# lamm-mit/MoleculeDiffusionTransformer

Hardware: AMD Instinct MI355X
Metric: molecules/sec @64 diffusion steps (QM9 max_len=64) (higher is better)
Workload: dtype f32 storage/accumulate; GEMM products as split-bf16 (bf16x3) MFMA; 1 GPU; QMDiffusion inverse sample(): channels=64 pred_dim=16 max_len=64 cond_len=12, batch=1024/GPU, 64 timesteps (126 U-Net evals), cond_scale=1.0, fp32; global_batch=1024, parallelism=batch-shard x1

## Files before the change

moleculediffusiontransformer_amd/csrc/k_tf256.hip:

```cpp
#include <cstdlib>
#include <type_traits>

#include "mdt_kernels.h"
#include "mdt_device.h"

#ifndef MDT_TF_F32
#define MDT_TF_F32 0
#endif

#ifndef MDT_KV_CPOL
#define MDT_KV_CPOL 2
#endif

namespace mdt {

namespace {

enum { K_T = 0, K_N = 1, K_O = 2 };
enum { D_P = 0, D_O = 1, D_K = 2, D_V = 3, D_SCRATCH = 4, D_SCRATCH_VEC = 5 };

template <int N>
__device__ __forceinline__ void frag_wait() {
#ifdef MDT_ABL_LGKM
  __builtin_amdgcn_sched_barrier(0);
#else
  lgkm_wait<N>();
#endif
}

constexpr int C = 256;
constexpr int CS = 128;
constexpr int SLOT = 256 * CS;
constexpr int NS = 4;
constexpr int IPT = CS / 16;
constexpr int NST = C / 32;
constexpr int NCT = C / 16;
constexpr int NU = 4;
constexpr int KTM = 3;
constexpr int RED_BYTES = KTM * 4 * 64 * 16;
constexpr int VEC_FLOATS = 768;
constexpr int VEC_BYTES = VEC_FLOATS * 4;
#ifndef MDT_XH_MODE
#define MDT_XH_MODE 0
#endif
#ifdef MDT_ABL_BAR
#define MDT_BARRIER() __builtin_amdgcn_sched_barrier(0)
#else
#define MDT_BARRIER() __builtin_amdgcn_s_barrier()
#endif
#ifndef MDT_STREAM_PF
#define MDT_STREAM_PF 8
#endif
#ifndef MDT_RING_AHEAD
#define MDT_RING_AHEAD 2
#endif
#ifndef MDT_XH_ADDR
#define MDT_XH_ADDR 1
#endif
constexpr int AUX_ST = MDT_XH_MODE == 1 ? 17 : (MDT_XH_MODE == 3 ? 18 : (MDT_XH_MODE == 4 ? 19 : 16));
constexpr int AUX_LD = MDT_XH_MODE == 0 ? 16 : (MDT_XH_MODE == 3 ? 18 : (MDT_XH_MODE == 4 ? 19 : 17));
constexpr unsigned XBLOCK = 32 * C * 4;
constexpr unsigned long long POLL_TIMEOUT = 30000000ull;

}

template <int NPW, int NSPLIT, bool F32>
__global__ __launch_bounds__(512) void k_tf256(TFArgs a) {
  extern __shared__ __attribute__((aligned(1024))) unsigned char smem[];
  unsigned char* red_b = smem + NS * SLOT;
  unsigned char* vec_b = red_b + RED_BYTES;

  const int tid = threadIdx.x, lane = tid & 63;
  const int wave = __builtin_amdgcn_readfirstlane(tid >> 6);
  const int NT = a.NT;
  const unsigned char* wsrc = reinterpret_cast<const unsigned char*>(a.w);
  int rb = blockIdx.x, hh = 0;
  const int nrb = (a.M + 31) / 32;
  if constexpr (NSPLIT == 2) {
    const int S = a.pair_stride, id = blockIdx.x;
    const int grp = id / (2 * S), w = id - grp * 2 * S;
    hh = w / S;
    rb = a.rb_base + grp * S + (w - hh * S);
    if (rb >= nrb) return;
  }

  if (wave >= 4) {
    const int iw = wave - 4;
    __builtin_amdgcn_s_setprio(MDT_LOADER_PRIO);
    const cu32p tiles = (cu32p)(a.tiles + (NSPLIT == 2 ? hh * NT : 0));
    const int lpP = lane >> 5;
    const int xP = (lane & 15) ^ lpP;
    const int baseP = ((lane >> 4) & 1) * (128 * CS) + lpP * (2 * CS);
    const int xO = (lane & 7) ^ (lane >> 4);
    const int baseO = (lane >> 3) * 128;
    unsigned voffP[IPT], voffO[IPT];
#pragma unroll
    for (int q = 0; q < IPT; ++q) {
      const int inst = iw + 4 * q;
      const int U = 2 * inst;
      voffP[q] = F32 ? (unsigned)(inst * 1024 + lane * 16) : (unsigned)(U * (2 * CS) + ((xP ^ (U & 15)) << 4) + baseP);
      voffO[q] = F32 ? (unsigned)(inst * 1024 + lane * 16)
                     : (unsigned)(((inst * 8) / CS) * (128 * CS) + ((inst * 8) % CS) * 128 + ((xO ^ (4 * (inst & 1))) << 4) + baseO);
    }
    const int sample0 = rb * (32 / a.T);
    const bool second = a.kv2 && sample0 >= a.nsamples / 2;
    unsigned voffKV[8];
    if constexpr (NPW > 0) {
      const int kv_rows = (32 / a.T) * a.Tk;
      const int bstr = second ? 0 : a.kv_bstride;
#pragma unroll
      for (int q = 0; q < NPW; ++q) {
        const int R = 4 * (iw + 4 * q) + (lane >> 4);
        const int Rc = min(R, kv_rows - 1);
        const int sm = min(Rc / a.Tk, a.nsamples - 1 - sample0), key = Rc % a.Tk;
        voffKV[q] = (unsigned)(((sm * bstr + key) * a.ldkv + 4 * ((lane & 15) ^ (R & 15))) * 4);
      }
    }
    auto pieces_of = [&](unsigned d) -> int {
      const unsigned kind = d & 7u;
      if (kind == D_SCRATCH) return 0;
      if (kind == D_SCRATCH_VEC) return iw < VEC_BYTES / 1024 ? 1 : 0;
      if (kind >= D_K) return NPW;
      return IPT;
    };
    auto issue_vec = [&](unsigned aux) {
      if (iw < VEC_BYTES / 1024)
        __builtin_amdgcn_global_load_lds(reinterpret_cast<const unsigned char*>(a.vec) + (aux >> 1) * 1024 + iw * 1024 + lane * 16,
                                         (__attribute__((address_space(3))) void*)(vec_b + (aux & 1u) * VEC_BYTES + iw * 1024), 16, 0, 0);
    };
    auto issue_tile = [&](int tau, unsigned d) {
      unsigned char* slot = smem + MDT_SLOT_IDX(tau) * SLOT + iw * 1024;
      const unsigned kind = d & 7u, aux = d >> 3;
      if (kind == D_SCRATCH) return;
      if (kind == D_SCRATCH_VEC) { issue_vec(aux); return; }
      if (kind >= D_K) {
        if constexpr (NPW > 0) {
          const int layer = (int)(aux >> 4), head = (int)(aux & 15u);
          const float* lb = second ? a.kv2 + (int64_t)layer * a.kv2_lstride
                                   : a.kv + (int64_t)layer * a.kv_lstride + (int64_t)sample0 * a.kv_bstride * a.ldkv;
          const unsigned char* base = reinterpret_cast<const unsigned char*>(lb + 64 * head + (kind == D_V ? 64 * a.nheads : 0));
#pragma unroll
          for (int q = 0; q < NPW; ++q)
            __builtin_amdgcn_global_load_lds(base + voffKV[q], (__attribute__((address_space(3))) void*)(slot + q * 4096), 16, 0, MDT_KV_CPOL);
        }
        return;
      }
      const unsigned char* tile = wsrc + (int64_t)aux * SLOT;
      const bool ptile = kind == D_P;
#pragma unroll
      for (int q = 0; q < IPT; ++q) {
        const unsigned off = ptile ? voffP[q] : voffO[q];
        __builtin_amdgcn_global_load_lds(tile + off, (__attribute__((address_space(3))) void*)(slot + q * 4096), 16, 0, 0);
      }
    };
    auto wait_vm = [&](int allow) {
#ifdef MDT_ABL_VMWAIT
      return;
#endif
      switch (allow) {
#define MDT_VMW(n) case n: asm volatile("s_waitcnt vmcnt(" #n ")" ::: "memory"); break;
        MDT_VMW(0) MDT_VMW(1) MDT_VMW(2) MDT_VMW(3) MDT_VMW(4) MDT_VMW(5) MDT_VMW(6) MDT_VMW(7) MDT_VMW(8) MDT_VMW(9) MDT_VMW(10)
        MDT_VMW(11) MDT_VMW(12) MDT_VMW(13) MDT_VMW(14) MDT_VMW(15)
#undef MDT_VMW
        default: asm volatile("s_waitcnt vmcnt(16)" ::: "memory"); break;
      }
    };
    constexpr int AHEAD = MDT_RING_AHEAD;
    unsigned dq[AHEAD];
    MDT_BARRIER();
    issue_vec(0u);
#pragma unroll
    for (int j = 0; j < AHEAD; ++j) {
      const unsigned d = j < NT ? tiles[j] : 0u;
      if (j < NT) issue_tile(j, d);
      if (j > 0) dq[j - 1] = d;
    }
    constexpr bool PF_ON = MDT_STREAM_PF > 0 && AHEAD == 2;
    const int pf_groups = PF_ON ? max(1, (int)gridDim.x / (8 * NSPLIT)) : 1;
    const int pf_mine = (int)blockIdx.x / (8 * NSPLIT);
    int pf_turn = MDT_STREAM_PF % pf_groups;
    unsigned char* pf_sink_b = vec_b + 2 * VEC_BYTES;
    int pf1 = 0, pf2 = 0;
    for (int k = 0; k < NT; ++k) {
      const unsigned dnew = k + AHEAD < NT ? tiles[k + AHEAD] : 0u;
      int allow = 0;
#pragma unroll
      for (int j = 0; j < AHEAD - 1; ++j) allow += k + 1 + j < NT ? pieces_of(dq[j]) : 0;
      if (PF_ON && k + 1 < NT) allow += pf1 + pf2;
      if (allow == IPT) asm volatile("s_waitcnt vmcnt(8)" ::: "memory");
      else if (NPW > 0 && allow == NPW) asm volatile("s_waitcnt vmcnt(%0)" ::"n"(NPW > 0 ? NPW : 1) : "memory");
      else wait_vm(allow);
      MDT_BARRIER();
      if (k + AHEAD < NT) issue_tile(k + AHEAD, dnew);
      if constexpr (PF_ON) {
        pf2 = pf1;
        pf1 = 0;
        const bool mine = pf_turn == pf_mine;
        if (++pf_turn == pf_groups) pf_turn = 0;
        if (mine && k + MDT_STREAM_PF < NT) {
          const unsigned dp = tiles[k + MDT_STREAM_PF];
          const unsigned kp = dp & 7u;
          if (kp != D_SCRATCH && kp != D_SCRATCH_VEC && kp < D_K) {
            const unsigned char* t = wsrc + (int64_t)(dp >> 3) * SLOT + (iw * 64 + lane) * 128;
            __builtin_amdgcn_global_load_lds(t, (__attribute__((address_space(3))) void*)(pf_sink_b + iw * 256), 4, 0, 0);
            pf1 = 1;
          }
        }
      }
#pragma unroll
      for (int j = 0; j + 1 < AHEAD - 1; ++j) dq[j] = dq[j + 1];
      dq[AHEAD - 2] = dnew;
    }
    prefetch_next_weights(a.pf_ptr, a.pf_lines, iw * 64 + lane);
    return;
  }

  const int i = lane & 15, g = lane >> 4;
  const int rt = wave >> 1, fh = wave & 1;
  const int row0 = rb * 32 + rt * 16;
  const int m = row0 + i;
  const bool mvalid = m < a.M;
  const int mc = mvalid ? m : a.M - 1;
  f32x4* red = reinterpret_cast<f32x4*>(red_b);

  f32x4 accT[NCT];
#ifdef MDT_STAMPS
  unsigned long long* stamps = reinterpret_cast<unsigned long long*>(a.xflags + 64 + 64 * nrb + 512 * hh);
  int nstamp = 0;
#define MDT_STAMP()                                                                                           \
  do {                                                                                                        \
    if (NSPLIT == 2 && rb == 0 && wave == 0 && nstamp < 250) {                                                \
      unsigned long long t_;                                                                                  \
      asm volatile("s_memtime %0\n\ts_waitcnt lgkmcnt(0)" : "=s"(t_)::"memory");                              \
      if (lane == 0) stamps[nstamp] = (t_ & 0xffffffffffffull) | ((unsigned long long)__LINE__ << 48);        \
      ++nstamp;                                                                                               \
    }                                                                                                         \
  } while (0)
#else
#define MDT_STAMP() do {} while (0)
#endif
#ifdef MDT_XH_LOG
  unsigned xlog_first = 0, xlog_last = 0, xlog_got = 0, xlog_epoch = 0;
#endif
  unsigned xround = 0;
  int xn = 0;
  __amdgpu_buffer_rsrc_t xres, fres;
  const unsigned fown = (64u + 32u * (unsigned)(2 * rb + hh)) * 4u;
  if constexpr (NSPLIT == 2) {
    xres = __builtin_amdgcn_make_buffer_rsrc(a.xbuf, 0, 0x7fffffff, 0x00020000);
    fres = __builtin_amdgcn_make_buffer_rsrc(a.xflags, 0, 0x7fffffff, 0x00020000);
    xround = (unsigned)__builtin_amdgcn_readfirstlane(__builtin_amdgcn_raw_buffer_load_b32(fres, fown, 0, AUX_LD));
  }
#ifdef MDT_XH_LOG
  xlog_epoch = xround;
#endif
  {
    const float* xp = a.x + (int64_t)mc * C + 4 * g;
    float4 xr[NCT];
#pragma unroll
    for (int ct = 0; ct < NCT; ++ct) xr[ct] = *reinterpret_cast<const float4*>(xp + 16 * ct);
    __builtin_amdgcn_sched_barrier(0);
    MDT_BARRIER();
    __builtin_amdgcn_sched_barrier(0);
#pragma unroll
    for (int ct = 0; ct < NCT; ++ct) accT[ct] = f32x4{xr[ct].x, xr[ct].y, xr[ct].z, xr[ct].w};
  }

  const int aP0 = F32 ? lane * 16 + fh * 16384 : fh * (2 * 16 * 4 * CS) + i * (4 * CS) + ((g ^ i) & 15) * 16;
  auto aP = [&](int st) -> int { return F32 ? aP0 : aP0 ^ (64 * st); };
  const int aO = F32 ? lane * 16 + fh * 2048 : i * 128 + ((4 * fh + g) ^ ((i >> 1) & 7)) * 16;

  bf16x8 frh[3][2], frl[3][2];
  auto frag_read = [&](auto kind, unsigned base, auto uc, int set, auto jc) {
    constexpr int KIND = decltype(kind)::value, u = decltype(uc)::value, j = decltype(jc)::value;
    constexpr int q = j >> 1, lo = j & 1;
    constexpr int off = F32 ? ((KIND == K_O) ? ((2 * u + q) * 4096 + lo * 1024) : (q * 8192 + u * 2048 + lo * 1024))
                            : ((KIND == K_O) ? ((2 * u + q) * 16 * 128 + lo * (CS * 128)) : (q * 16 * 4 * CS + lo * (2 * CS)));
#ifdef MDT_ABL_LDSBC
    lds_read16_off<off>(lo ? frl[set][q] : frh[set][q], base & 0x18000u);
#else
    if constexpr (F32) lds_read16_off<off>(frh[set][q], base);
    else lds_read16_off<off>(lo ? frl[set][q] : frh[set][q], base);
#endif
  };
  using J0 = std::integral_constant<int, 0>;
  using J1 = std::integral_constant<int, 1>;
  using J2 = std::integral_constant<int, 2>;
  using J3 = std::integral_constant<int, 3>;
  unsigned pb2 = 0, pb3 = 0;
  auto prefetch2 = [&](auto kind, const unsigned char* slot, int off) {
    constexpr int KIND = decltype(kind)::value;
    const unsigned l = lds_addr(slot);
    if constexpr (F32) {
      const unsigned b = l + (KIND == K_O ? aO : aP0);
      frag_read(kind, b, J0{}, 0, J0{}); frag_read(kind, b, J0{}, 0, J2{});
      return;
    }
    const unsigned b0 = l + (KIND == K_O ? aO : aP(0)), b1 = l + (KIND == K_O ? aO : aP(1));
    pb2 = l + (KIND == K_O ? aO : aP(2));
    pb3 = l + (KIND == K_O ? aO : aP(3));
    frag_read(kind, b0, J0{}, off % 3, J0{}); frag_read(kind, b0, J0{}, off % 3, J1{});
    frag_read(kind, b0, J0{}, off % 3, J2{}); frag_read(kind, b0, J0{}, off % 3, J3{});
    frag_read(kind, b1, J1{}, (off + 1) % 3, J0{}); frag_read(kind, b1, J1{}, (off + 1) % 3, J1{});
    frag_read(kind, b1, J1{}, (off + 1) % 3, J2{}); frag_read(kind, b1, J1{}, (off + 1) % 3, J3{});
  };

  int tau = 0;
  auto slot_of = [&](int t) -> unsigned char* { return smem + MDT_SLOT_IDX(t) * SLOT; };
  auto lane_now = [&]() -> int {
    if constexpr (F32) return lane;
    int l = (int)__builtin_amdgcn_mbcnt_hi(~0u, __builtin_amdgcn_mbcnt_lo(~0u, 0u));
    asm volatile("" : "+v"(l));
    return l;
  };

  auto phase = [&](auto kind, auto offc, auto nkind, bool has_next, f32x4* acc, const bf16x8* bh, const bf16x8* bl) {
    constexpr int KIND = decltype(kind)::value, OFF = decltype(offc)::value, NK = decltype(nkind)::value;
    if constexpr (F32) {
      const unsigned lc = lds_addr(slot_of(tau)) + (KIND == K_O ? aO : aP0);
      const unsigned lnx = lds_addr(slot_of(tau + 1)) + (NK == K_O ? aO : aP0);
      auto half32 = [&](auto vc) {
        constexpr int v = decltype(vc)::value, u = v >> 1, hl = v & 1;
        if (v == 2 * NU - 1 && has_next) {
          __builtin_amdgcn_sched_barrier(0);
          MDT_BARRIER();
          __builtin_amdgcn_sched_barrier(0);
        }
        frag_wait<0>();
        constexpr int s0 = v & 1, s1 = (v + 1) & 1;
        constexpr bool in_phase = v + 1 < 2 * NU;
        const bool pre = in_phase || has_next;
        constexpr int ia = (KIND == K_O) ? 2 * u : 0, ib = (KIND == K_O) ? 0 : u;
        auto rd = [&](auto qc) {
          if (!pre) return;
          constexpr int q = decltype(qc)::value;
          __builtin_amdgcn_sched_barrier(0);
          constexpr int un = (v + 1) / 2, jn = 2 * q + ((v + 1) & 1);
          if constexpr (in_phase) frag_read(kind, lc, std::integral_constant<int, un>{}, s1, std::integral_constant<int, jn>{});
          else frag_read(nkind, lnx, std::integral_constant<int, 0>{}, s1, std::integral_constant<int, 2 * q>{});
          __builtin_amdgcn_sched_barrier(0);
        };
        const f32x4 a0 = __builtin_bit_cast(f32x4, frh[s0][0]), a1 = __builtin_bit_cast(f32x4, frh[s0][1]);
        const f32x4 xb = __builtin_bit_cast(f32x4, hl ? bl[ib] : bh[ib]);
        auto mm2 = [&](auto r0c) {
          constexpr int r0 = decltype(r0c)::value;
#pragma unroll
          for (int r = r0; r < r0 + 2; ++r) {
            if constexpr (KIND == K_N) {
              acc[ia] = MDT_MFMA_F32(xb[r], a0[r], acc[ia], 0, 0, 0);
              acc[ia + 1] = MDT_MFMA_F32(xb[r], a1[r], acc[ia + 1], 0, 0, 0);
            } else {
              acc[ia] = MDT_MFMA_F32(a0[r], xb[r], acc[ia], 0, 0, 0);
              acc[ia + 1] = MDT_MFMA_F32(a1[r], xb[r], acc[ia + 1], 0, 0, 0);
            }
          }
        };
        mm2(J0{}); rd(J0{});
        mm2(J2{}); rd(J1{});
        __builtin_amdgcn_sched_barrier(0);
      };
      half32(std::integral_constant<int, 0>{}); half32(std::integral_constant<int, 1>{});
      half32(std::integral_constant<int, 2>{}); half32(std::integral_constant<int, 3>{});
      half32(std::integral_constant<int, 4>{}); half32(std::integral_constant<int, 5>{});
      half32(std::integral_constant<int, 6>{}); half32(std::integral_constant<int, 7>{});
      ++tau;
      return;
    }
    unsigned ln = 0, bn[2] = {0u, 0u};
    auto unit = [&](auto uc) {
      constexpr int u = decltype(uc)::value;
      if (u == NU - 2 && has_next) {
        __builtin_amdgcn_sched_barrier(0);
#ifndef MDT_RING_NODRAIN
        if constexpr (MDT_RING_AHEAD >= 3) asm volatile("s_waitcnt lgkmcnt(0)" ::: "memory");
#endif
        MDT_BARRIER();
#ifdef MDT_STAGGER
        if (fh) { for (int d_ = 0; d_ < MDT_STAGGER; ++d_) asm volatile("s_nop 15" ::: "memory"); }
#endif
        __builtin_amdgcn_sched_barrier(0);
      }
      constexpr int s0 = (OFF + u) % 3, s2 = (OFF + u + 2) % 3;
      constexpr bool in_phase = u + 2 < NU;
      const bool pre = in_phase || has_next;
      const bool later = (u + 1 < NU) || has_next;
      if (later) frag_wait<4>(); else frag_wait<0>();
      constexpr int ia = (KIND == K_O) ? 2 * u : 0, ib = (KIND == K_O) ? 0 : u;
      auto rd = [&](auto jc) {
        if (!pre) return;
        __builtin_amdgcn_sched_barrier(0);
        if constexpr (in_phase) frag_read(kind, u == 0 ? pb2 : pb3, std::integral_constant<int, u + 2>{}, s2, jc);
        else frag_read(nkind, bn[u + 2 - NU], std::integral_constant<int, u + 2 - NU>{}, s2, jc);
        __builtin_amdgcn_sched_barrier(0);
      };
      auto mm = [&](const bf16x8& w, const bf16x8& x, int q) {
        if constexpr (KIND == K_N) acc[ia + q] = MDT_MFMA_BF16(x, w, acc[ia + q], 0, 0, 0);
        else acc[ia + q] = MDT_MFMA_BF16(w, x, acc[ia + q], 0, 0, 0);
      };
      mm(frl[s0][0], bh[ib], 0); rd(J0{});
      mm(frl[s0][1], bh[ib], 1); rd(J1{});
      mm(frh[s0][0], bl[ib], 0); rd(J2{});
      mm(frh[s0][1], bl[ib], 1); rd(J3{});
      mm(frh[s0][0], bh[ib], 0);
      if constexpr (u == 1) {
        __builtin_amdgcn_sched_barrier(0);
        ln = lds_addr(slot_of(tau + 1));
        bn[0] = ln + (NK == K_O ? aO : aP(0));
        bn[1] = ln + (NK == K_O ? aO : aP(1));
        __builtin_amdgcn_sched_barrier(0);
      }
      if constexpr (u == NU - 1) {
        __builtin_amdgcn_sched_barrier(0);
        pb2 = ln + (NK == K_O ? aO : aP(2));
        pb3 = ln + (NK == K_O ? aO : aP(3));
        __builtin_amdgcn_sched_barrier(0);
      }
      mm(frh[s0][1], bh[ib], 1);
      __builtin_amdgcn_sched_barrier(0);
    };
    unit(std::integral_constant<int, 0>{}); unit(std::integral_constant<int, 1>{});
    unit(std::integral_constant<int, 2>{}); unit(std::integral_constant<int, 3>{});
    ++tau;
  };
  using IC0 = std::integral_constant<int, 0>;
  using IC1 = std::integral_constant<int, 1>;
  using IC2 = std::integral_constant<int, 2>;
  const IC0 kT{};
  const IC1 kN{};
  const IC2 kO{};

  const float scale2 = a.scale * 1.44269504088896340736f;
  const int nkeys = NPW > 0 ? (16 / a.T) * a.Tk : 0;
  const int tsh = __builtin_ctz((unsigned)a.T);
  auto self_mask = [&](int l) -> unsigned {
    const int sq = (l & 15) >> tsh, g4 = 4 * (l >> 4);
    unsigned kb = 0;
#pragma unroll
    for (int r = 0; r < 4; ++r) kb |= (((g4 + r) >> tsh) == sq) ? (1u << r) : 0u;
    return kb;
  };
  auto cross_consts = [&](int l, unsigned& kb0, unsigned (&vb0)[4], unsigned& okbits) {
    const int i_ = l & 15, g_ = l >> 4;
    const int Rw = rt * nkeys;
    kb0 = (unsigned)((Rw + i_) * 256 + (((8 * fh + g_) ^ ((Rw + i_) & 15)) << 4));
#pragma unroll
    for (int r = 0; r < 4; ++r) {
      const int R = Rw + 4 * g_ + r;
      vb0[r] = (unsigned)(R * 256 + (i_ & 3) * 4 + (((8 * fh + (i_ >> 2)) ^ (R & 15)) << 4));
    }
    const int k_lo = (i_ >> tsh) * a.Tk, k_hi = k_lo + a.Tk;
    okbits = 0;
#pragma unroll
    for (int kt = 0; kt < KTM; ++kt)
#pragma unroll
      for (int r = 0; r < 4; ++r) {
        const int jj = 16 * kt + 4 * g_ + r;
        if (jj >= k_lo && jj < k_hi) okbits |= 1u << (4 * kt + r);
      }
  };
  unsigned kbits = 0, kb0 = 0, vb0[4] = {0, 0, 0, 0}, okbits = 0;
  if constexpr (F32) {
    kbits = self_mask(lane);
    if constexpr (NPW > 0) cross_consts(lane, kb0, vb0, okbits);
  }
  const f32x4 zero4 = f32x4{0.f, 0.f, 0.f, 0.f};
  const float t1 = a.T > 1 ? 1.f : 0.f, t2 = a.T > 2 ? 1.f : 0.f, t4 = a.T > 4 ? 1.f : 0.f, t8 = a.T > 8 ? 1.f : 0.f;
  auto dpp_fma = [](float v, float f, auto ctrl) {
    const int mm_ = __builtin_amdgcn_update_dpp(0, __builtin_bit_cast(int, v), decltype(ctrl)::value, 0xf, 0xf, true);
    return __builtin_fmaf(__builtin_bit_cast(float, mm_), f, v);
  };
  auto token_sum = [&](float (&s)[NCT]) {
#pragma unroll
    for (int ct = 0; ct < NCT; ++ct) s[ct] = dpp_fma(s[ct], t1, std::integral_constant<int, 0xB1>{});
#pragma unroll
    for (int ct = 0; ct < NCT; ++ct) s[ct] = dpp_fma(s[ct], t2, std::integral_constant<int, 0x4E>{});
#pragma unroll
    for (int ct = 0; ct < NCT; ++ct) s[ct] = dpp_fma(s[ct], t4, std::integral_constant<int, 0x141>{});
#pragma unroll
    for (int ct = 0; ct < NCT; ++ct) s[ct] = dpp_fma(s[ct], t8, std::integral_constant<int, 0x140>{});
  };

  MDT_STAMP();
  asm volatile("s_waitcnt vmcnt(0) lgkmcnt(0)" ::: "memory");
  MDT_STAMP();
  MDT_BARRIER();
  prefetch2(kT, slot_of(0), 0);
  const unsigned vec_l0 = lds_addr(vec_b);
  int vpar = 0;

  bf16x8 xh[NST], xl[NST];
  auto make_operands = [&](bool layernorm) {
    float mean = 0.f, rstd = 1.f;
    if (layernorm) {
      float s = 0.f;
#pragma unroll
      for (int ct = 0; ct < NCT; ++ct) s += (accT[ct][0] + accT[ct][1]) + (accT[ct][2] + accT[ct][3]);
      s = xg16_add(s);
      s = xg32_add(s);
      mean = s / (float)C;
      float ss = 0.f;
#pragma unroll
      for (int ct = 0; ct < NCT; ++ct)
#pragma unroll
        for (int r = 0; r < 4; ++r) {
          const float d = accT[ct][r] - mean;
          ss += d * d;
        }
      ss = xg16_add(ss);
      ss = xg32_add(ss);
      rstd = 1.0f / sqrtf(ss / (float)C + a.eps_ln);
    }
#pragma unroll
    for (int st = 0; st < NST; ++st) {
      float v[8];
#pragma unroll
      for (int e = 0; e < 8; ++e) v[e] = mvalid ? (accT[2 * st + (e >> 2)][e & 3] - mean) * rstd : 0.f;
      split8<F32>(v, xh[st], xl[st]);
    }
  };
  auto start_acc = [&](int off, bool keep_residual) {
    const float* p = reinterpret_cast<const float*>(vec_b + vpar * VEC_BYTES) + off + 4 * (lane_now() >> 4);
#pragma unroll
    for (int ct = 0; ct < NCT; ++ct) {
      const float4 b = *reinterpret_cast<const float4*>(p + 16 * ct);
      const f32x4 bb = f32x4{b.x, b.y, b.z, b.w};
      const f32x4 mine = keep_residual ? accT[ct] + bb : bb;
      accT[ct] = (fh | hh) ? zero4 : mine;
    }
  };
  auto exchange_half = [&](auto rdc) {
    constexpr int rd_ = decltype(rdc)::value;
    f32x4* ex = reinterpret_cast<f32x4*>(slot_of(tau)) + lane_now();
#pragma unroll
    for (int c = 0; c < 8; ++c) ex[(wave * 8 + c) * 64] = accT[8 * rd_ + c];
    asm volatile("s_waitcnt lgkmcnt(0)" ::: "memory");
    MDT_BARRIER();
#pragma unroll
    for (int c = 0; c < 8; ++c) {
      const f32x4 other = ex[((wave ^ 1) * 8 + c) * 64];
      accT[8 * rd_ + c] = fh ? (other + accT[8 * rd_ + c]) : (accT[8 * rd_ + c] + other);
    }
    asm volatile("s_waitcnt lgkmcnt(0)" ::: "memory");
    ++tau;
  };
  auto pair_handoff = [&]() {
    if constexpr (NSPLIT == 2) {
      const unsigned sbase = __builtin_amdgcn_readfirstlane(
          (((unsigned)(xn & 1) * (unsigned)nrb + (unsigned)rb) * 2u + (unsigned)hh) * XBLOCK + (unsigned)rt * (16u * 1024u));
      const unsigned vlane = (unsigned)lane_now() * 16u;
#pragma unroll
      for (int c = 0; c < 8; ++c) {
        const f32x4 lo_ = accT[c], hi_ = accT[8 + c];
        const f32x4 v = f32x4{fh ? hi_[0] : lo_[0], fh ? hi_[1] : lo_[1], fh ? hi_[2] : lo_[2], fh ? hi_[3] : lo_[3]};
#if MDT_XH_ADDR
        __builtin_amdgcn_raw_buffer_store_b128(__builtin_bit_cast(i32x4, v), xres, vlane + sbase + (unsigned)(8 * fh + c) * 1024u, 0, AUX_ST);
#else
        __builtin_amdgcn_raw_buffer_store_b128(__builtin_bit_cast(i32x4, v), xres, vlane, sbase + (unsigned)(8 * fh + c) * 1024u, AUX_ST);
#endif
      }
      MDT_STAMP();
      asm volatile("s_waitcnt vmcnt(0)" ::: "memory");
      MDT_STAMP();
      MDT_BARRIER();
      MDT_STAMP();
      ++xround;
      if (wave == 0) {
        __builtin_amdgcn_raw_buffer_store_b32((int)xround, fres, fown, 0, AUX_ST);
        const unsigned long long t0 = __builtin_amdgcn_s_memrealtime();
#ifdef MDT_XH_LOG
        int xtries = 0;
#endif
        for (;;) {
#ifdef MDT_XH_LOG
          ++xtries;
#endif
          asm volatile("" ::: "memory");
          const unsigned got = (unsigned)__builtin_amdgcn_raw_buffer_load_b32(fres, fown ^ 128u, 0, AUX_LD);
          if ((int)(got - xround) >= 0) {
#ifdef MDT_XH_LOG
            if (xtries == 1) ++xlog_first;
            xlog_got = got;
#endif
            break;
          }
          __builtin_amdgcn_s_sleep(2);
          if (__builtin_amdgcn_s_memrealtime() - t0 > POLL_TIMEOUT) {
            if (lane_now() == 0) atomicOr(a.xflags, 1u);
            break;
          }
        }
      }
      MDT_STAMP();
#ifdef MDT_XH_D2
      if (wave == 0) for (int d = 0; d < 40; ++d) __builtin_amdgcn_s_sleep(127);
#endif
      MDT_BARRIER();
      asm volatile("" ::: "memory");
      const unsigned sother = sbase ^ XBLOCK;
#pragma unroll
      for (int half = 0; half < 2; ++half) {
        f32x4 o[8];
#pragma unroll
        for (int c = 0; c < 8; ++c)
#if MDT_XH_ADDR
          o[c] = __builtin_bit_cast(f32x4, __builtin_amdgcn_raw_buffer_load_b128(xres, vlane + sother + (unsigned)(8 * half + c) * 1024u, 0,
                                                                                 AUX_LD));
#else
          o[c] = __builtin_bit_cast(f32x4, __builtin_amdgcn_raw_buffer_load_b128(xres, vlane, sother + (unsigned)(8 * half + c) * 1024u,
                                                                                 AUX_LD));
#endif
#pragma unroll
        for (int c = 0; c < 8; ++c) accT[8 * half + c] = hh ? (o[c] + accT[8 * half + c]) : (accT[8 * half + c] + o[c]);
      }
      ++xn;
      tau += 2;
#ifdef MDT_XH_LOG
      xlog_last = xround;
#endif
      MDT_STAMP();
    }
  };
  auto exchange = [&]() {
    MDT_STAMP();
    exchange_half(std::integral_constant<int, 0>{});
    exchange_half(std::integral_constant<int, 1>{});
    vpar ^= 1;
    MDT_STAMP();
    pair_handoff();
  };
  auto next_subblock = [&]() {
    MDT_BARRIER();
    prefetch2(kT, slot_of(tau), 0);
    MDT_STAMP();
  };

  if (a.has_in) {
    float gm[NCT], gv[NCT];
#pragma unroll
    for (int ct = 0; ct < NCT; ++ct) gm[ct] = xg16_add((accT[ct][0] + accT[ct][1]) + (accT[ct][2] + accT[ct][3]));
    token_sum(gm);
    const float inv_n = 1.0f / (float)(8 * a.T);
#pragma unroll
    for (int ct = 0; ct < NCT; ++ct) {
      gm[ct] *= inv_n;
      float ss = 0.f;
#pragma unroll
      for (int r = 0; r < 4; ++r) {
        const float d = accT[ct][r] - gm[ct];
        ss += d * d;
      }
      gv[ct] = xg16_add(ss);
    }
    token_sum(gv);
#pragma unroll
    for (int ct = 0; ct < NCT; ++ct) {
      const float rs = __builtin_amdgcn_rsqf(gv[ct] * inv_n + a.eps_gn);
#pragma unroll
      for (int r = 0; r < 4; ++r) accT[ct][r] = (accT[ct][r] - gm[ct]) * rs;
    }
    make_operands(false);
    const float* bp = reinterpret_cast<const float*>(vec_b + vpar * VEC_BYTES) + 4 * (lane_now() >> 4);
    if constexpr (NSPLIT == 1) {
      auto in_chunk = [&](auto cc, auto o0, auto o1, bool more) {
        constexpr int c = decltype(cc)::value;
        f32x4 t[2] = {zero4, zero4};
        phase(kT, o0, kT, true, t, xh, xl);
        phase(kT, o1, kT, more, t, xh + 4, xl + 4);
#pragma unroll
        for (int q = 0; q < 4; ++q) {
          const float4 b = *reinterpret_cast<const float4*>(bp + 16 * (4 * c + q));
          const f32x4 bb = fh ? zero4 : f32x4{b.x, b.y, b.z, b.w};
          const f32x4 mine = (q >> 1) == 0 ? (fh ? zero4 : t[q & 1]) : (fh ? t[q & 1] : zero4);
          accT[4 * c + q] = mine + bb;
        }
      };
      in_chunk(IC0{}, IC0{}, IC1{}, true);
      in_chunk(IC1{}, IC2{}, IC0{}, true);
      in_chunk(IC2{}, IC1{}, IC2{}, true);
      in_chunk(std::integral_constant<int, 3>{}, IC0{}, IC1{}, false);
    } else {
      f32x4 t0[2] = {zero4, zero4}, t1[2] = {zero4, zero4};
      phase(kT, IC0{}, kT, true, t0, xh, xl);
      phase(kT, IC1{}, kT, true, t0, xh + 4, xl + 4);
      phase(kT, IC2{}, kT, true, t1, xh, xl);
      phase(kT, IC0{}, kT, false, t1, xh + 4, xl + 4);
#pragma unroll
      for (int ct = 0; ct < NCT; ++ct) {
        const int hv = ct >> 3, j = (ct >> 2) & 1, fv = (ct >> 1) & 1, q = ct & 1;
        const float4 b = *reinterpret_cast<const float4*>(bp + 16 * ct);
        const bool own = (hh == hv) && (fh == fv);
        const f32x4 tv = j ? t1[q] : t0[q];
        const bool first = (hh | fh) == 0;
#pragma unroll
        for (int r = 0; r < 4; ++r) {
          const float bias_r = r == 0 ? b.x : (r == 1 ? b.y : (r == 2 ? b.z : b.w));
          accT[ct][r] = (own ? tv[r] : 0.f) + (first ? bias_r : 0.f);
        }
      }
    }
    exchange();
    next_subblock();
  }

  const int nheads = a.nheads / NSPLIT, nff = a.nff / NSPLIT;
  const int h0 = hh * nheads, f0 = hh * nff;
  for (int blk = 0; blk < a.nblocks; ++blk) {
    const bool last_blk = blk + 1 == a.nblocks;
    const unsigned bias_l = 128u * (unsigned)fh + 16u * (unsigned)(lane_now() >> 4);
    {
      make_operands(true);
      start_acc(64 * a.nheads, true);
      MDT_STAMP();
      const unsigned bl = vec_l0 + vpar * VEC_BYTES + bias_l + 256u * (unsigned)h0;
      for (int h = 0; h < nheads; ++h) {
        const bool more = h + 1 < nheads;
        f32x4 oT[2];
        f32x4 qT[2], kTt[2], vT[2];
#pragma unroll
        for (int q = 0; q < 2; ++q) { kTt[q] = zero4; vT[q] = zero4; qT[q] = zero4; }
#ifdef MDT_STAMPS_HEAD
#define MDT_HSTAMP() do { if (blk == 0) MDT_STAMP(); } while (0)
#else
#define MDT_HSTAMP() do {} while (0)
#endif
        phase(kT, IC0{}, kT, true, qT, xh, xl);
        MDT_HSTAMP();
        phase(kT, IC1{}, kT, true, qT, xh + 4, xl + 4);
        MDT_HSTAMP();
        phase(kT, IC2{}, kT, true, kTt, xh, xl);
        MDT_HSTAMP();
        phase(kT, IC0{}, kN, true, kTt, xh + 4, xl + 4);
        MDT_HSTAMP();
        phase(kN, IC1{}, kN, true, vT, xh, xl);
        MDT_HSTAMP();
        phase(kN, IC2{}, kN, false, vT, xh + 4, xl + 4);
        MDT_HSTAMP();
        {
          f32x4 bq[2];
          lds_read_f4_off<0>(bq[0], bl + 256 * h); lds_read_f4_off<64>(bq[1], bl + 256 * h);
          frag_wait<0>();
          qT[0] += bq[0];
          qT[1] += bq[1];
        }
        f32x4 sp0 = zero4, sp1 = zero4;
#pragma unroll
        for (int r = 0; r < 4; ++r) {
          sp0 = MDT_MFMA_F32(kTt[0][r], qT[0][r], sp0, 0, 0, 0);
          sp1 = MDT_MFMA_F32(kTt[1][r], qT[1][r], sp1, 0, 0, 0);
        }
        const f32x4 mine = sp0 + sp1;
        f32x4* redl = red + lane_now();
        redl[wave * 64] = mine;
        asm volatile("s_waitcnt lgkmcnt(0)" ::: "memory");
        MDT_BARRIER();
        const f32x4 other = redl[(wave ^ 1) * 64];
        prefetch2(kO, slot_of(tau), 1);
        const f32x4 s01 = fh ? (other + mine) : (mine + other);
        f32x4 st;
        float mx = -INFINITY;
        if constexpr (!F32) kbits = self_mask(lane_now());
#pragma unroll
        for (int r = 0; r < 4; ++r) {
          const float sv = ((kbits >> r) & 1u) ? s01[r] * scale2 : -INFINITY;
          st[r] = sv;
          mx = fmaxf(mx, sv);
        }
        mx = xg16_max(mx);
        mx = xg32_max(mx);
        float sum = 0.f;
#pragma unroll
        for (int r = 0; r < 4; ++r) {
          const float e = __builtin_amdgcn_exp2f(st[r] - mx);
          st[r] = e;
          sum += e;
        }
        sum = xg16_add(sum);
        sum = xg32_add(sum);
        const float inv = __builtin_amdgcn_rcpf(sum);
        oT[0] = zero4; oT[1] = zero4;
#pragma unroll
        for (int r = 0; r < 4; ++r) {
          const float p = st[r] * inv;
          oT[0] = MDT_MFMA_F32(vT[0][r], p, oT[0], 0, 0, 0);
          oT[1] = MDT_MFMA_F32(vT[1][r], p, oT[1], 0, 0, 0);
        }
        bf16x8 oh[1], ol[1];
        {
          float v[8];
#pragma unroll
          for (int e = 0; e < 8; ++e) v[e] = oT[e >> 2][e & 3];
          split8<F32>(v, oh[0], ol[0]);
        }
        MDT_HSTAMP();
        phase(kO, IC1{}, kO, true, accT, oh, ol);
        MDT_HSTAMP();
        phase(kO, IC2{}, kT, more, accT + 8, oh, ol);
        MDT_HSTAMP();
      }
      exchange();
      next_subblock();
    }
    if constexpr (NPW > 0) {
      make_operands(true);
      start_acc(64 * a.nheads, true);
      MDT_STAMP();
      const unsigned bl = vec_l0 + vpar * VEC_BYTES + bias_l + 256u * (unsigned)h0;
      for (int h = 0; h < nheads; ++h) {
        const bool more = h + 1 < nheads;
        f32x4 oT[2];
        f32x4 qT[2];
        qT[0] = zero4; qT[1] = zero4;
        phase(kT, IC0{}, kT, true, qT, xh, xl);
        phase(kT, IC1{}, kT, false, qT, xh + 4, xl + 4);
        MDT_BARRIER();
        const unsigned char* sk = slot_of(tau);
        if constexpr (!F32) cross_consts(lane_now(), kb0, vb0, okbits);
        {
          f32x4 bq[2];
          lds_read_f4_off<0>(bq[0], bl + 256 * h); lds_read_f4_off<64>(bq[1], bl + 256 * h);
          frag_wait<0>();
          qT[0] += bq[0];
          qT[1] += bq[1];
        }
        f32x4 st[KTM];
        float4 k0[KTM], k1[KTM];
#pragma unroll
        for (int kt = 0; kt < KTM; ++kt) {
          k0[kt] = *reinterpret_cast<const float4*>(sk + kb0 + 4096 * kt);
          k1[kt] = *reinterpret_cast<const float4*>(sk + (kb0 ^ 64u) + 4096 * kt);
        }
        f32x4 sp0[KTM], sp1[KTM];
#pragma unroll
        for (int kt = 0; kt < KTM; ++kt) { sp0[kt] = zero4; sp1[kt] = zero4; }
#pragma unroll
        for (int kt = 0; kt < KTM; ++kt) { sp0[kt] = MDT_MFMA_F32(k0[kt].x, qT[0][0], sp0[kt], 0, 0, 0); sp1[kt] = MDT_MFMA_F32(k1[kt].x, qT[1][0], sp1[kt], 0, 0, 0); }
#pragma unroll
        for (int kt = 0; kt < KTM; ++kt) { sp0[kt] = MDT_MFMA_F32(k0[kt].y, qT[0][1], sp0[kt], 0, 0, 0); sp1[kt] = MDT_MFMA_F32(k1[kt].y, qT[1][1], sp1[kt], 0, 0, 0); }
#pragma unroll
        for (int kt = 0; kt < KTM; ++kt) { sp0[kt] = MDT_MFMA_F32(k0[kt].z, qT[0][2], sp0[kt], 0, 0, 0); sp1[kt] = MDT_MFMA_F32(k1[kt].z, qT[1][2], sp1[kt], 0, 0, 0); }
#pragma unroll
        for (int kt = 0; kt < KTM; ++kt) { sp0[kt] = MDT_MFMA_F32(k0[kt].w, qT[0][3], sp0[kt], 0, 0, 0); sp1[kt] = MDT_MFMA_F32(k1[kt].w, qT[1][3], sp1[kt], 0, 0, 0); }
        f32x4* redl = red + lane_now();
#pragma unroll
        for (int kt = 0; kt < KTM; ++kt) {
          st[kt] = sp0[kt] + sp1[kt];
          redl[(kt * 4 + wave) * 64] = st[kt];
        }
        asm volatile("s_waitcnt lgkmcnt(0)" ::: "memory");
        ++tau;
        MDT_BARRIER();
        const unsigned char* sv = slot_of(tau);
        float mx = -INFINITY;
#pragma unroll
        for (int kt = 0; kt < KTM; ++kt) {
          const f32x4 other = redl[(kt * 4 + (wave ^ 1)) * 64];
          const f32x4 s01 = fh ? (other + st[kt]) : (st[kt] + other);
#pragma unroll
          for (int r = 0; r < 4; ++r) {
            const float sv2 = ((okbits >> (4 * kt + r)) & 1u) ? s01[r] * scale2 : -INFINITY;
            st[kt][r] = sv2;
            mx = fmaxf(mx, sv2);
          }
        }
        mx = xg16_max(mx);
        mx = xg32_max(mx);
        float sum = 0.f;
#pragma unroll
        for (int kt = 0; kt < KTM; ++kt)
#pragma unroll
          for (int r = 0; r < 4; ++r) {
            const float e = __builtin_amdgcn_exp2f(st[kt][r] - mx);
            st[kt][r] = e;
            sum += e;
          }
        sum = xg16_add(sum);
        sum = xg32_add(sum);
        const float inv = __builtin_amdgcn_rcpf(sum);
        oT[0] = zero4; oT[1] = zero4;
        f32x4 v0[KTM], v1[KTM];
#pragma unroll
        for (int kt = 0; kt < KTM; ++kt)
#pragma unroll
          for (int r = 0; r < 4; ++r) {
            v0[kt][r] = *reinterpret_cast<const float*>(sv + vb0[r] + 4096 * kt);
            v1[kt][r] = *reinterpret_cast<const float*>(sv + (vb0[r] ^ 64u) + 4096 * kt);
          }
#pragma unroll
        for (int kt = 0; kt < KTM; ++kt)
#pragma unroll
          for (int r = 0; r < 4; ++r) {
            const float p = st[kt][r] * inv;
            oT[0] = MDT_MFMA_F32(v0[kt][r], p, oT[0], 0, 0, 0);
            oT[1] = MDT_MFMA_F32(v1[kt][r], p, oT[1], 0, 0, 0);
          }
        asm volatile("s_waitcnt lgkmcnt(0)" ::: "memory");
        ++tau;
        MDT_BARRIER();
        prefetch2(kO, slot_of(tau), 1);
        bf16x8 oh[1], ol[1];
        {
          float v[8];
#pragma unroll
          for (int e = 0; e < 8; ++e) v[e] = oT[e >> 2][e & 3];
          split8<F32>(v, oh[0], ol[0]);
        }
        phase(kO, IC1{}, kO, true, accT, oh, ol);
        phase(kO, IC2{}, kT, more, accT + 8, oh, ol);
      }
      exchange();
      next_subblock();
    }
    {
      const int npost = last_blk ? a.npost : 0;
      make_operands(false);
      start_acc(64 * a.nff, npost == 0);
      MDT_STAMP();
      const unsigned bl = vec_l0 + vpar * VEC_BYTES + bias_l + 256u * (unsigned)f0;
      for (int h = 0; h < nff; ++h) {
        const bool more = h + 1 < nff;
        f32x4 oT[2];
        oT[0] = zero4; oT[1] = zero4;
        phase(kT, IC0{}, kT, true, oT, xh, xl);
        phase(kT, IC1{}, kT, false, oT, xh + 4, xl + 4);
        MDT_BARRIER();
        prefetch2(kO, slot_of(tau), 1);
        {
          f32x4 b1[2];
          lds_read_f4_off<0>(b1[0], bl + 256 * h); lds_read_f4_off<64>(b1[1], bl + 256 * h);
          frag_wait<0>();
#pragma unroll
          for (int q = 0; q < 2; ++q)
#pragma unroll
            for (int r = 0; r < 4; ++r) oT[q][r] = gelu(oT[q][r] + b1[q][r]);
        }
        bf16x8 oh[1], ol[1];
        {
          float v[8];
#pragma unroll
          for (int e = 0; e < 8; ++e) v[e] = oT[e >> 2][e & 3];
          split8<F32>(v, oh[0], ol[0]);
        }
        phase(kO, IC1{}, kO, true, accT, oh, ol);
        if (npost > 0 && !more) phase(kO, IC2{}, kO, true, accT + 8, oh, ol);
        else phase(kO, IC2{}, kT, more, accT + 8, oh, ol);
      }
      if (npost > 0) {
        bf16x8 oxh[1], oxl[1];
        auto pick = [&](int kc) {
          const i32x4 h0v = __builtin_bit_cast(i32x4, xh[2 * kc]), h1v = __builtin_bit_cast(i32x4, xh[2 * kc + 1]);
          const i32x4 l0v = __builtin_bit_cast(i32x4, xl[2 * kc]), l1v = __builtin_bit_cast(i32x4, xl[2 * kc + 1]);
          i32x4 hv, lv;
#pragma unroll
          for (int k = 0; k < 4; ++k) { hv[k] = fh ? h1v[k] : h0v[k]; lv[k] = fh ? l1v[k] : l0v[k]; }
          oxh[0] = __builtin_bit_cast(bf16x8, hv);
          oxl[0] = __builtin_bit_cast(bf16x8, lv);
        };
        if constexpr (NSPLIT == 1) {
          pick(0); phase(kO, IC0{}, kO, true, accT, oxh, oxl); phase(kO, IC1{}, kO, true, accT + 8, oxh, oxl);
          pick(1); phase(kO, IC2{}, kO, true, accT, oxh, oxl); phase(kO, IC0{}, kO, true, accT + 8, oxh, oxl);
          pick(2); phase(kO, IC1{}, kO, true, accT, oxh, oxl); phase(kO, IC2{}, kO, true, accT + 8, oxh, oxl);
          pick(3); phase(kO, IC0{}, kO, true, accT, oxh, oxl); phase(kO, IC1{}, kT, false, accT + 8, oxh, oxl);
        } else {
          auto pick2 = [&](int j) {
            const i32x4 a0 = __builtin_bit_cast(i32x4, xh[2 * j]), a1 = __builtin_bit_cast(i32x4, xh[2 * j + 1]);
            const i32x4 a2 = __builtin_bit_cast(i32x4, xh[4 + 2 * j]), a3 = __builtin_bit_cast(i32x4, xh[5 + 2 * j]);
            const i32x4 b0 = __builtin_bit_cast(i32x4, xl[2 * j]), b1 = __builtin_bit_cast(i32x4, xl[2 * j + 1]);
            const i32x4 b2 = __builtin_bit_cast(i32x4, xl[4 + 2 * j]), b3 = __builtin_bit_cast(i32x4, xl[5 + 2 * j]);
            i32x4 hv, lv;
#pragma unroll
            for (int k = 0; k < 4; ++k) {
              hv[k] = hh ? (fh ? a3[k] : a2[k]) : (fh ? a1[k] : a0[k]);
              lv[k] = hh ? (fh ? b3[k] : b2[k]) : (fh ? b1[k] : b0[k]);
            }
            oxh[0] = __builtin_bit_cast(bf16x8, hv);
            oxl[0] = __builtin_bit_cast(bf16x8, lv);
          };
          pick2(0); phase(kO, IC0{}, kO, true, accT, oxh, oxl); phase(kO, IC1{}, kO, true, accT + 8, oxh, oxl);
          pick2(1); phase(kO, IC2{}, kO, true, accT, oxh, oxl); phase(kO, IC0{}, kT, false, accT + 8, oxh, oxl);
        }
      }
      exchange();
      if (!last_blk) next_subblock();
    }
  }

  MDT_STAMP();
#ifdef MDT_XH_LOG
  if (NSPLIT == 2 && wave == 0 && lane == 0 && rb < 4) {
    unsigned* lg = a.xflags + 64 + 64 * nrb + 4096 * (2 * rb + hh);
    const unsigned slot = atomicAdd(lg, 1u);
    if (slot < 500) {
      unsigned xcc;
      asm volatile("s_getreg_b32 %0, hwreg(HW_REG_XCC_ID)" : "=s"(xcc));
      unsigned* e = lg + 8 + 8 * slot;
      e[0] = xlog_epoch; e[1] = xcc & 15u; e[2] = xlog_first; e[3] = xlog_got; e[4] = xlog_last; e[5] = blockIdx.x;
    }
  }
#endif
  const int ln_end = lane_now();
  const int m_end = rb * 32 + rt * 16 + (ln_end & 15);
  if (m_end < a.M) {
    if constexpr (NSPLIT == 1) {
      float* xo = a.out + (int64_t)m_end * C + 4 * (ln_end >> 4) + 128 * fh;
#pragma unroll
      for (int c = 0; c < 8; ++c) {
        const f32x4 lo_ = accT[c], hi_ = accT[8 + c];
        store_nt(xo + 16 * c, make_float4(fh ? hi_[0] : lo_[0], fh ? hi_[1] : lo_[1], fh ? hi_[2] : lo_[2], fh ? hi_[3] : lo_[3]));
      }
    } else {
      float* xo = a.out + (int64_t)m_end * C + 4 * (ln_end >> 4) + 128 * fh + 64 * hh;
#pragma unroll
      for (int c = 0; c < 4; ++c) {
        const f32x4 q0 = accT[c], q1 = accT[4 + c], q2 = accT[8 + c], q3 = accT[12 + c];
        float v[4];
#pragma unroll
        for (int r = 0; r < 4; ++r) v[r] = fh ? (hh ? q3[r] : q2[r]) : (hh ? q1[r] : q0[r]);
        store_nt(xo + 16 * c, make_float4(v[0], v[1], v[2], v[3]));
      }
    }
  }
}

#if MDT_TF_F32
extern int g_pair_capacity_override;
#else
int g_pair_capacity_override = 0;
#endif

template <int NPW, int NSPLIT, bool F32>
static hipError_t launch_tf2(const TFArgs& a, hipStream_t s) {
  const size_t smem = (size_t)NS * SLOT + RED_BYTES + 2 * VEC_BYTES + 1024;
  static DevOnce attr_once;
  if (attr_once.first()) {
    (void)hipFuncSetAttribute(reinterpret_cast<const void*>(&k_tf256<NPW, NSPLIT, F32>), hipFuncAttributeMaxDynamicSharedMemorySize,
                              (int)(160 * 1024));
  }
  const int nrb = (a.M + 31) / 32;
  if constexpr (NSPLIT == 1) {
    hipLaunchKernelGGL((k_tf256<NPW, NSPLIT, F32>), dim3((unsigned)nrb), dim3(512), smem, s, a);
    return hipGetLastError();
  } else {
    static int cap_of[64] = {0};
    int dev = 0;
    if (hipGetDevice(&dev) != hipSuccess || dev < 0 || dev >= 64) return hipErrorInvalidDevice;
    if (cap_of[dev] == 0) {
      int cus = 0, per_cu = 0;
      if (hipDeviceGetAttribute(&cus, hipDeviceAttributeMultiprocessorCount, dev) != hipSuccess) return hipErrorInvalidDevice;
      if (hipOccupancyMaxActiveBlocksPerMultiprocessor(&per_cu, reinterpret_cast<const void*>(&k_tf256<NPW, NSPLIT, F32>), 512, smem) != hipSuccess)
        return hipErrorInvalidValue;
      cap_of[dev] = cus * per_cu > 0 ? cus * per_cu : -1;
    }
    const int S = a.pair_stride;
    const int groups_fit = g_pair_capacity_override > 0 ? g_pair_capacity_override / (2 * S) : cap_of[dev] / (2 * S);
    if (groups_fit < 1) return hipErrorLaunchOutOfResources;
    const int ngroups = (nrb + S - 1) / S;
    for (int g0 = 0; g0 < ngroups; g0 += groups_fit) {
      TFArgs b = a;
      b.rb_base = g0 * S;
      const int ng = ngroups - g0 < groups_fit ? ngroups - g0 : groups_fit;
      hipLaunchKernelGGL((k_tf256<NPW, NSPLIT, F32>), dim3(2u * (unsigned)S * (unsigned)ng), dim3(512), smem, s, b);
      const hipError_t e = hipGetLastError();
      if (e != hipSuccess) return e;
    }
    return hipSuccess;
  }
}

template <int NSPLIT>
static hipError_t launch_tf256_n(const TFArgs& a, hipStream_t s) {
  constexpr bool kF32 = MDT_TF_F32 != 0;
  const bool cross = a.kv != nullptr;
  if (!cross) return launch_tf2<0, NSPLIT, kF32>(a, s);
  switch (((32 / a.T) * a.Tk + 15) / 16) {
    case 1: return launch_tf2<1, NSPLIT, kF32>(a, s);
    case 2: return launch_tf2<2, NSPLIT, kF32>(a, s);
    case 3: return launch_tf2<3, NSPLIT, kF32>(a, s);
    case 4: return launch_tf2<4, NSPLIT, kF32>(a, s);
    case 5: return launch_tf2<5, NSPLIT, kF32>(a, s);
    case 6: return launch_tf2<6, NSPLIT, kF32>(a, s);
    default: return hipErrorInvalidValue;
  }
}

#if MDT_TF_F32
hipError_t launch_tf256_f32(const TFArgs& a, hipStream_t s) {
#else
int tf256_pair_capacity() {
  if (g_pair_capacity_override > 0) return g_pair_capacity_override;
  int dev = 0, cus = 0, per_cu = 0;
  if (hipGetDevice(&dev) != hipSuccess) return 0;
  if (hipDeviceGetAttribute(&cus, hipDeviceAttributeMultiprocessorCount, dev) != hipSuccess) return 0;
  const size_t smem = (size_t)NS * SLOT + RED_BYTES + 2 * VEC_BYTES + 1024;
  (void)hipFuncSetAttribute(reinterpret_cast<const void*>(&k_tf256<6, 2, false>), hipFuncAttributeMaxDynamicSharedMemorySize, (int)(160 * 1024));
  if (hipOccupancyMaxActiveBlocksPerMultiprocessor(&per_cu, reinterpret_cast<const void*>(&k_tf256<6, 2, false>), 512, smem) != hipSuccess) return 0;
  return cus * per_cu;
}

bool tf256_supported(int T, int Tk, int nheads, int nff, bool cross) {
  if (T <= 0 || 16 % T || nheads != 8 || nff != 8) return false;
  if (cross && (Tk <= 0 || (16 / T) * Tk > 48)) return false;
  return true;
}

hipError_t launch_tf256(const TFArgs& a, hipStream_t s) {
  if (a.wf32) return launch_tf256_f32(a, s);
#endif
  if (a.M <= 0) return hipSuccess;
  const bool cross = a.kv != nullptr;
  if (!tf256_supported(a.T, a.Tk, a.nheads, a.nff, cross) || a.nblocks <= 0 || a.NT <= 0) return hipErrorInvalidValue;
  if (a.npost != 0 && a.npost != 8) return hipErrorInvalidValue;
  if (a.nsplit == 2) {
    if (!a.xbuf || !a.xflags || a.pair_stride <= 0 || a.pair_stride > 64) return hipErrorInvalidValue;
    return launch_tf256_n<2>(a, s);
  }
  return launch_tf256_n<1>(a, s);
}

}
```

Baseline: 4667 molecules/s.

## Restructure split-K exchange as reduce-scatter, then start global handoff before all-gather

In the non-F32 path, each wave of a pair now reduces only its own feature half through LDS. It then stores that half to the cross-block handoff buffer, and a second LDS round copies the reduced half back to its partner. This replaces two full add-exchanges followed by a select-and-store, and lets the global stores be issued earlier so they overlap with the second LDS round. The aim is to cut redundant adds and select work and to hide store latency. The cost is more code paths and some duplication, and the F32 build keeps the old ordering.

```diff
diff --git a/moleculediffusiontransformer_amd/csrc/k_tf256.hip b/moleculediffusiontransformer_amd/csrc/k_tf256.hip
--- a/moleculediffusiontransformer_amd/csrc/k_tf256.hip
+++ b/moleculediffusiontransformer_amd/csrc/k_tf256.hip
@@ -528,37 +528,82 @@
       accT[ct] = (fh | hh) ? zero4 : mine;
     }
   };
-  auto exchange_half = [&](auto rdc) {
-    constexpr int rd_ = decltype(rdc)::value;
-    f32x4* ex = reinterpret_cast<f32x4*>(slot_of(tau)) + lane_now();
-#pragma unroll
-    for (int c = 0; c < 8; ++c) ex[(wave * 8 + c) * 64] = accT[8 * rd_ + c];
-    asm volatile("s_waitcnt lgkmcnt(0)" ::: "memory");
-    MDT_BARRIER();
-#pragma unroll
-    for (int c = 0; c < 8; ++c) {
-      const f32x4 other = ex[((wave ^ 1) * 8 + c) * 64];
-      accT[8 * rd_ + c] = fh ? (other + accT[8 * rd_ + c]) : (accT[8 * rd_ + c] + other);
-    }
-    asm volatile("s_waitcnt lgkmcnt(0)" ::: "memory");
-    ++tau;
-  };
-  auto pair_handoff = [&]() {
+  auto handoff_base = [&](int half) -> unsigned {
+    return __builtin_amdgcn_readfirstlane(
+        (((unsigned)(xn & 1) * (unsigned)nrb + (unsigned)rb) * 2u + (unsigned)half) * XBLOCK + (unsigned)rt * (16u * 1024u));
+  };
+  auto handoff_store = [&](const f32x4& v, unsigned vlane, unsigned sbase, unsigned tile) {
+#if MDT_XH_ADDR
+    __builtin_amdgcn_raw_buffer_store_b128(__builtin_bit_cast(i32x4, v), xres, vlane + sbase + tile * 1024u, 0, AUX_ST);
+#else
+    __builtin_amdgcn_raw_buffer_store_b128(__builtin_bit_cast(i32x4, v), xres, vlane, sbase + tile * 1024u, AUX_ST);
+#endif
+  };
+  auto exchange_as = [&](auto fhc) {
+    constexpr int own = 8 * decltype(fhc)::value, oth = 8 - own;
+    {
+      f32x4* ex = reinterpret_cast<f32x4*>(slot_of(tau)) + lane_now();
+#pragma unroll
+      for (int c = 0; c < 8; ++c) ex[(wave * 8 + c) * 64] = accT[oth + c];
+      asm volatile("s_waitcnt lgkmcnt(0)" ::: "memory");
+      MDT_BARRIER();
+#pragma unroll
+      for (int c = 0; c < 8; ++c) {
+        const f32x4 other = ex[((wave ^ 1) * 8 + c) * 64];
+        accT[own + c] = own ? (other + accT[own + c]) : (accT[own + c] + other);
+      }
+      asm volatile("s_waitcnt lgkmcnt(0)" ::: "memory");
+      ++tau;
+    }
+    MDT_STAMP();
     if constexpr (NSPLIT == 2) {
-      const unsigned sbase = __builtin_amdgcn_readfirstlane(
-          (((unsigned)(xn & 1) * (unsigned)nrb + (unsigned)rb) * 2u + (unsigned)hh) * XBLOCK + (unsigned)rt * (16u * 1024u));
-      const unsigned vlane = (unsigned)lane_now() * 16u;
+      const unsigned sbase = handoff_base(hh), vlane = (unsigned)lane_now() * 16u;
+#pragma unroll
+      for (int c = 0; c < 8; ++c) handoff_store(accT[own + c], vlane, sbase, (unsigned)(own + c));
+      MDT_STAMP();
+    }
+    {
+      f32x4* ex = reinterpret_cast<f32x4*>(slot_of(tau)) + lane_now();
+#pragma unroll
+      for (int c = 0; c < 8; ++c) ex[(wave * 8 + c) * 64] = accT[own + c];
+      asm volatile("s_waitcnt lgkmcnt(0)" ::: "memory");
+      MDT_BARRIER();
+#pragma unroll
+      for (int c = 0; c < 8; ++c) accT[oth + c] = ex[((wave ^ 1) * 8 + c) * 64];
+      asm volatile("s_waitcnt lgkmcnt(0)" ::: "memory");
+      ++tau;
+    }
+  };
+  auto exchange_both = [&]() {
+#pragma unroll
+    for (int rd_ = 0; rd_ < 2; ++rd_) {
+      f32x4* ex = reinterpret_cast<f32x4*>(slot_of(tau)) + lane_now();
+#pragma unroll
+      for (int c = 0; c < 8; ++c) ex[(wave * 8 + c) * 64] = accT[8 * rd_ + c];
+      asm volatile("s_waitcnt lgkmcnt(0)" ::: "memory");
+      MDT_BARRIER();
+#pragma unroll
+      for (int c = 0; c < 8; ++c) {
+        const f32x4 other = ex[((wave ^ 1) * 8 + c) * 64];
+        accT[8 * rd_ + c] = fh ? (other + accT[8 * rd_ + c]) : (accT[8 * rd_ + c] + other);
+      }
+      asm volatile("s_waitcnt lgkmcnt(0)" ::: "memory");
+      ++tau;
+    }
+    if constexpr (NSPLIT == 2) {
+      const unsigned sbase = handoff_base(hh), vlane = (unsigned)lane_now() * 16u;
 #pragma unroll
       for (int c = 0; c < 8; ++c) {
         const f32x4 lo_ = accT[c], hi_ = accT[8 + c];
         const f32x4 v = f32x4{fh ? hi_[0] : lo_[0], fh ? hi_[1] : lo_[1], fh ? hi_[2] : lo_[2], fh ? hi_[3] : lo_[3]};
-#if MDT_XH_ADDR
-        __builtin_amdgcn_raw_buffer_store_b128(__builtin_bit_cast(i32x4, v), xres, vlane + sbase + (unsigned)(8 * fh + c) * 1024u, 0, AUX_ST);
-#else
-        __builtin_amdgcn_raw_buffer_store_b128(__builtin_bit_cast(i32x4, v), xres, vlane, sbase + (unsigned)(8 * fh + c) * 1024u, AUX_ST);
-#endif
+        handoff_store(v, vlane, sbase, (unsigned)(8 * fh + c));
       }
       MDT_STAMP();
+    }
+  };
+  auto pair_handoff = [&]() {
+    if constexpr (NSPLIT == 2) {
+      const unsigned vlane = (unsigned)lane_now() * 16u;
       asm volatile("s_waitcnt vmcnt(0)" ::: "memory");
       MDT_STAMP();
       MDT_BARRIER();
@@ -596,7 +641,7 @@
 #endif
       MDT_BARRIER();
       asm volatile("" ::: "memory");
-      const unsigned sother = sbase ^ XBLOCK;
+      const unsigned sother = handoff_base(hh ^ 1);
 #pragma unroll
       for (int half = 0; half < 2; ++half) {
         f32x4 o[8];
@@ -622,8 +667,17 @@
   };
   auto exchange = [&]() {
     MDT_STAMP();
-    exchange_half(std::integral_constant<int, 0>{});
-    exchange_half(std::integral_constant<int, 1>{});
+    if constexpr (F32) {
+      exchange_both();
+    } else if (fh) {
+      asm volatile("; exchange as feature half 1" ::: "memory");
+      exchange_as(std::integral_constant<int, 1>{});
+      asm volatile("; exchanged as feature half 1" ::: "memory");
+    } else {
+      asm volatile("; exchange as feature half 0" ::: "memory");
+      exchange_as(std::integral_constant<int, 0>{});
+      asm volatile("; exchanged as feature half 0" ::: "memory");
+    }
     vpar ^= 1;
     MDT_STAMP();
     pair_handoff();
```

Measured after the change: 4688 molecules/s (median of 6 runs). No clear change (+0.4%).
